# tnibler/sift-features

Hardware: AMD Instinct MI355X
Metric: keypoints+descriptors/sec on 1920×1080 batch; HBM GB/s on pyramid stage (higher is better)
Workload: dtype f32; 1 GPU; batch of 128 x 1920x1080 u8 frames per GPU (configs[3] shard), full sift(); frames_per_gpu=128, frame=1920x1080, octaves=10, parallelism=dp1 (frames sharded, no collective)

## Files before the change

### sift-features_amd/csrc/pyramid.hip

```cpp
#include "launch_ext.h"
#include "sift_common.h"
#include "sift_kernels.h"

#include <algorithm>
#include <cstdlib>
#include <cstring>

namespace siftmi {

template <int R, int TH_, int QW_ = 8>
struct BlurGeom {
    static constexpr int TW = 64;
    static constexpr int TH = TH_;
    static constexpr int QW = QW_;
    static constexpr int HWL = (R + 3) & ~3;
    static constexpr int IH = TH + 2 * R;
    static constexpr int IWV = TW + 2 * HWL;
    static constexpr int IWP = IWV + 4;
    static constexpr int OFF = HWL - R;
    static constexpr int NV = (HWL + R + QW + 3) / 4;
    static constexpr int THP = IWP;
    static constexpr int LDS_FLOATS = IH * IWP;
    static constexpr int NLOAD4 = IH * (IWV / 4);
    static constexpr int LOADS_PER_THREAD = (NLOAD4 + 255) / 256;
// ... 332 lines not shown
            const f2v kr = {taps.k[R], taps.k[R]};
            acc = v[o] * kr;
#pragma unroll
            for (int t = 1; t <= 2 * R; t++) {
                const float k = taps.k[t > R ? t - R : R - t];
                const f2v kt = {k, k};
                acc = acc + v[o + t] * kt;
            }
        }
        out[o] = acc;
    }
    const int y0 = y + WV * G::VB;
    const int nrow = min(G::VB, ye - y0);
    const int gx = x0 + 2 * lane;
    const uint32_t lane_col = (uint32_t)(gx * 4), lane_bad = gx < W ? 0u : kStoreDrop;
    const uint32_t lane_ncol = (uint32_t)((gx >> 1) * 4);
    const uint32_t lane_nbad = ((gx >> 1) < wn && (P == kProfileOpenCV || gx + 1 < W)) ? 0u : kStoreDrop;
#pragma unroll
    for (int o = 0; o < G::VB; o++) {
        const int gy = y0 + o;
        const uint32_t row_bad = o < nrow ? 0u : kStoreDrop;
        __builtin_amdgcn_raw_buffer_store_b64(__builtin_bit_cast(u32x2, out[o]), rd,
                                              ((uint32_t)(gy * pitch * 4) + lane_col) | lane_bad | row_bad, 0,
                                              SIFT_STORE_CPOL);
        if (NXT && (o & 1) == (P == kProfileOpenCV ? 0 : 1)) {
            const uint32_t nrow_bad = (gy >> 1) < hn ? row_bad : kStoreDrop;
            const uint32_t odd = __builtin_bit_cast(u32x2, out[o]).y;
            const uint32_t val = P == kProfileOpenCV
                                     ? __builtin_bit_cast(u32x2, out[o]).x
                                     : __builtin_bit_cast(uint32_t, ip_unit_clamp(__builtin_bit_cast(float, odd)));
            __builtin_amdgcn_raw_buffer_store_b32(val, rn,
                                                  ((uint32_t)((gy >> 1) * pitch_n * 4) + lane_ncol) | lane_nbad |
                                                      nrow_bad,
                                                  0, 0);
        }
    }
}

template <class G, bool NXT = false, int LOFF = 0>
__device__ __forceinline__ void strip_colpass_clamped(const float* sa, const float* sb, const BlurTaps& taps,
                                                      int lane, int wv, int y, int ye, int x0, int W, int H,
                                                      int pitch, __amdgpu_buffer_rsrc_t rd,
                                                      __amdgpu_buffer_rsrc_t rn, int pitch_n, int wn, int hn) {
    constexpr int R = G::R;
    const int y0 = y + wv * G::VB;
    const int nrow = min(G::VB, ye - y0);
    const int gx = x0 + 2 * lane;
    const uint32_t lane_col = (uint32_t)(gx * 4), lane_bad = gx < W ? 0u : kStoreDrop;
    const uint32_t lane_ncol = (uint32_t)((gx >> 1) * 4);
    const uint32_t lane_nbad = ((gx >> 1) < wn && gx + 1 < W) ? 0u : kStoreDrop;
    for (int o = 0; o < G::VB; o++) {
        const int gy = y0 + o;
        f2v acc = {0.0f, 0.0f};
#pragma unroll
        for (int t = 0; t <= 2 * R; t++) {
            const int L = min(max(gy - R + t, 0), H - 1) - (y - R - LOFF);
            const float* rp = L < G::S ? sa + L * G::IWP : sb + (L - G::S) * G::IWP;
            const f2v v = *(const lds_f2v*)(rp + 2 * lane);
            const float k = taps.k[t > R ? t - R : R - t];
            const f2v kt = {k, k};
            acc = t == 0 ? v * kt : acc + v * kt;
        }
        const uint32_t row_bad = o < nrow ? 0u : kStoreDrop;
        __builtin_amdgcn_raw_buffer_store_b64(__builtin_bit_cast(u32x2, acc), rd,
                                              ((uint32_t)(gy * pitch * 4) + lane_col) | lane_bad | row_bad, 0,
                                              SIFT_STORE_CPOL);
        if (NXT && (gy & 1) == 1) {
            const uint32_t nrow_bad = (gy >> 1) < hn ? row_bad : kStoreDrop;
            __builtin_amdgcn_raw_buffer_store_b32(__builtin_bit_cast(uint32_t, ip_unit_clamp(__builtin_bit_cast(
                                                      float, __builtin_bit_cast(u32x2, acc).y))), rn,
                                                  ((uint32_t)((gy >> 1) * pitch_n * 4) + lane_ncol) | lane_nbad |
                                                      nrow_bad,
                                                  0, 0);
        }
    }
}

#ifndef SIFT_STRIP_NXT_MINB
#define SIFT_STRIP_NXT_MINB 3
#endif
template <int R, bool NXT>
constexpr int strip_minb() {
    return (NXT && R >= 7 && StripGeom<R>::MINB > SIFT_STRIP_NXT_MINB) ? SIFT_STRIP_NXT_MINB : StripGeom<R>::MINB;
}

template <int R, int P, bool NXT>
__global__ __launch_bounds__(256, (strip_minb<R, NXT>())) void k_blur_strip(
    const float* __restrict__ src, size_t src_img_stride, float* __restrict__ dst, size_t dst_img_stride,
    float* __restrict__ nxt, size_t nxt_img_stride, int pitch_n, int wn, int hn, int W, int H, int pitch,
    const BlurTaps taps, int ya, int yb, int seg) {
    using G = StripGeom<R>;
    static_assert(G::NCW == 2, "two chunk slots");
    __shared__ __attribute__((aligned(16))) float lds[G::LDS_FLOATS];
    const int tid = threadIdx.x, lane = tid & 63;
    const int wv = __builtin_amdgcn_readfirstlane(tid >> 6);
    const TileId tile = xcd_tile();
    const int x0 = tile.x * G::TW;
    const int ys = ya + tile.y * seg, ye = min(yb, ys + seg);
    if (ys >= ye) return;
    const size_t b = tile.z;
    const uint32_t plane_bytes = (uint32_t)H * (uint32_t)pitch * 4u;
    const __amdgpu_buffer_rsrc_t rs = uniform_rsrc(src + b * src_img_stride, plane_bytes);
    const __amdgpu_buffer_rsrc_t rd = uniform_rsrc(dst + b * dst_img_stride, plane_bytes);
    __amdgpu_buffer_rsrc_t rn = rd;
    if constexpr (NXT) rn = uniform_rsrc(nxt + b * nxt_img_stride, (uint32_t)hn * (uint32_t)pitch_n * 4u);
    const bool cols_in = x0 - G::HWL >= 0 && x0 + G::TW + G::HWL <= W;
    int voff[G::LPT];
#pragma unroll
    for (int j = 0; j < G::LPT; j++) {
        const int i = min(tid + 64 * G::NW * j, G::NLOAD4 - 1);
        const int ly = i / G::C4, c4 = i - ly * G::C4;
        voff[j] = (ly * pitch + x0 - G::HWL + 4 * c4) * 4;
    }
    int prow, pq;
    strip_rowpass_map(lane, wv, prow, pq);
    const int nsteps = (ye - ys + G::S - 1) / G::S;
    float4 pre[G::LPT];
    strip_load<R, P>(pre, rs, voff, cols_in, ys - R, x0, W, H, pitch);
    strip_store<G>(pre, lds);
    strip_load<R, P>(pre, rs, voff, cols_in, ys - R + G::S, x0, W, H, pitch);
    drop_stores<G::VB * (NXT ? 2 : 1)>(rd);
    __syncthreads();
    strip_rowpass<G, P>(lds, taps, prow, pq);
    for (int k = 0; k < nsteps; k++) {
        float* sa = lds + (k & 1) * G::SLOT;
        float* sb = lds + ((k + 1) & 1) * G::SLOT;
        __syncthreads();
        strip_store<G>(pre, sb);
        if (k + 2 <= nsteps) strip_load<R, P>(pre, rs, voff, cols_in, ys - R + (k + 2) * G::S, x0, W, H, pitch);
        __syncthreads();
        strip_rowpass<G, P>(sb, taps, prow, pq);
        __syncthreads();
        const int y = ys + k * G::S;
        switch (wv) {
#define COLPASS(w)                                                                                      \
    case w:                                                                                             \
        strip_colpass<G, P, w, NXT>(sa, sb, taps, lane, y, ye, x0, W, pitch, rd, rn, pitch_n, wn, hn); \
        break;
            COLPASS(0) COLPASS(1) COLPASS(2) COLPASS(3)
            default:
                __builtin_unreachable();
#undef COLPASS
        }
    }
}

template <int Ra, int Rb, int HA = -1>
struct PairGeom {
    using GA = StripGeom<Ra, 16, HA>;
    using GB = StripGeom<Rb, 16>;
    static constexpr int HB = GB::HWL;
    static constexpr int TWO = GA::TW - 2 * HB;
    static constexpr int NBW = GB::NCW;
    static constexpr int NBR = NBW + 1;
    static constexpr int LDS_FLOATS = 2 * GA::SLOT + NBR * GB::SLOT;
    static constexpr int MINB = 163840 / (4 * LDS_FLOATS + 2048) < 4 ? 163840 / (4 * LDS_FLOATS + 2048) : 4;
    static_assert(GA::HWL <= 8 && GA::NCW == 2, "A: radius <= 8");
    static_assert(NBW == 2, "B: radius <= 8 (two-chunk column windows)");
    static_assert(GB::IWV >= GA::TW, "B's window holds A's 128 columns");
};

template <class GA, int WV, bool NXT, int P = kProfileOpenCV>
__device__ __forceinline__ void pair_colpass_a(const float* sa, const float* sb, float* bslot, int bip,
                                               const BlurTaps& taps, int lane, int y, int gys, int gye, int xa,
                                               int hb, int W, int pitch, int two, __amdgpu_buffer_rsrc_t rd,
                                               __amdgpu_buffer_rsrc_t rn, int pitch_n, int wn, int hn) {
    constexpr int R = GA::R;
    constexpr int NR = GA::VB + 2 * R;
    f2v v[NR];
#pragma unroll
    for (int j = 0; j < NR; j++) {
        const int L = WV * GA::VB + j;
        const float* rp = L < GA::S ? sa + L * GA::IWP : sb + (L - GA::S) * GA::IWP;
        v[j] = *(const lds_f2v*)(rp + 2 * lane);
    }
    const f2v k0 = {taps.k[0], taps.k[0]};
    const int y0 = y + WV * GA::VB;
    const int gx = xa + 2 * lane;
    const bool own = gx >= xa + hb && gx < xa + hb + two && gx < W;
    const uint32_t colbad = own ? 0u : kStoreDrop;

#pragma unroll
    for (int o = 0; o < GA::VB; o++) {
        f2v acc;
        if constexpr (P == kProfileOpenCV) {
            acc = v[o + R] * k0;
#pragma unroll
            for (int t = 1; t <= R; t++) {
                const f2v kt = {taps.k[t], taps.k[t]};
                acc = __builtin_elementwise_fma(v[o + R + t] + v[o + R - t], kt, acc);
            }
        } else {
            const f2v kr = {taps.k[R], taps.k[R]};
            acc = v[o] * kr;
#pragma unroll
            for (int t = 1; t <= 2 * R; t++) {
                const float k = taps.k[t > R ? t - R : R - t];
                const f2v kt = {k, k};
                acc = acc + v[o + t] * kt;
            }
        }
        *(f2v*)(bslot + (WV * GA::VB + o) * bip + 2 * lane) = acc;
        const int gy = y0 + o;
        const uint32_t rowbad = gy >= gys && gy < gye ? 0u : kStoreDrop;
        const uint32_t off = (uint32_t)((gy * pitch + gx) * 4);
        __builtin_amdgcn_raw_buffer_store_b64(__builtin_bit_cast(u32x2, acc), rd, off | colbad | rowbad, 0,
                                              SIFT_STORE_CPOL);
        if constexpr (NXT) {
            const uint32_t nbad = (gy & 1) == 0 && (gy >> 1) < hn ? rowbad : kStoreDrop;
            const uint32_t ncol = (gx >> 1) < wn ? colbad : kStoreDrop;
            __builtin_amdgcn_raw_buffer_store_b32(__builtin_bit_cast(uint32_t, acc.x), rn,
                                                  (uint32_t)(((gy >> 1) * pitch_n + (gx >> 1)) * 4) | ncol | nbad, 0,
                                                  0);
        }
    }
}

template <int Ra, int P, class GA>
struct PlaneIn {
    float4 pre[GA::LPT];
    __amdgpu_buffer_rsrc_t rs;
    int voff[GA::LPT];
    bool cols_in;
    int xa, W, H, pitch;
    __device__ __forceinline__ void init(const float* src, int xa_, int W_, int H_, int pitch_) {
        xa = xa_, W = W_, H = H_, pitch = pitch_;
        rs = uniform_rsrc(src, (uint32_t)H * (uint32_t)pitch * 4u);
        cols_in = xa - GA::HWL >= 0 && xa + GA::TW + GA::HWL <= W;
        const int tid = threadIdx.x;
#pragma unroll
        for (int j = 0; j < GA::LPT; j++) {
            const int i = min(tid + 64 * GA::NW * j, GA::NLOAD4 - 1);
            const int ly = i / GA::C4, c4 = i - ly * GA::C4;
            voff[j] = (ly * pitch + xa - GA::HWL + 4 * c4) * 4;
        }
    }
    __device__ __forceinline__ void prefetch(int r0) { strip_load<Ra, P, GA>(pre, rs, voff, cols_in, r0, xa, W, H, pitch); }
    __device__ __forceinline__ void store(float* slot, int) { strip_store<GA>(pre, slot); }
};

template <int Ra, int Rb, bool NXT, int P, bool NXTB, int LOFF, int HA, class AIn>
__device__ __forceinline__ void blur2_body(AIn& ain, float* lds, __amdgpu_buffer_rsrc_t ra, __amdgpu_buffer_rsrc_t rb,
                                           __amdgpu_buffer_rsrc_t rn, int pitch_n, int wn, int hn, int X, int ys,
                                           int ye, int W, int H, int pitch, const BlurTaps& taps_a,
                                           const BlurTaps& taps_b) {
    using Q = PairGeom<Ra, Rb, HA>;
    using GA = typename Q::GA;
    using GB = typename Q::GB;
    constexpr int S = GA::S;
    constexpr int NBW = Q::NBW, NBR = Q::NBR;
    static_assert(!(NXT && NXTB), "one next-octave output");
    float* aslot = lds;
    float* bslot = lds + 2 * GA::SLOT;
    const int tid = threadIdx.x, lane = tid & 63;
    const int wv = __builtin_amdgcn_readfirstlane(tid >> 6);
    const int xa = X - Q::HB;
    int prow, pq;
    strip_rowpass_map(lane, wv, prow, pq);
    const bool fix_l = xa < 0, fix_r = xa + GA::TW > W;
    auto fixup = [&](float* slot) {
        if (!(fix_l || fix_r)) return;
        constexpr int NE = 4 * 2 * Q::HB, NIT = (NE + 63) / 64;
        float val[NIT];
        bool act[NIT];
        int dst[NIT];
#pragma unroll
        for (int it = 0; it < NIT; it++) {
            const int e = lane + 64 * it;
            const int r = wv * 4 + e / (2 * Q::HB), j = e % (2 * Q::HB);
            const int x = j < Q::HB ? xa + j : W + (j - Q::HB);
            act[it] = e < NE && (j < Q::HB ? (fix_l && x < 0) : (fix_r && x - xa < GA::TW));
            dst[it] = r * GB::IWP + (x - xa);
            const int sx = P == kProfileOpenCV ? reflect101(x, W) : clamp_idx(x, W);
            val[it] = act[it] ? slot[r * GB::IWP + (sx - xa)] : 0.0f;
        }
        __builtin_amdgcn_fence(__ATOMIC_RELEASE, "wavefront");
        __builtin_amdgcn_wave_barrier();
#pragma unroll
        for (int it = 0; it < NIT; it++)
            if (act[it]) slot[dst[it]] = val[it];
        __builtin_amdgcn_fence(__ATOMIC_RELEASE, "wavefront");
        __builtin_amdgcn_wave_barrier();
    };
    const int nout = (ye - ys + S - 1) / S;
    const int ng = nout + NBW - 2, na = ng + 1;
    const int ga = ys - Rb - Ra - LOFF;
    ain.prefetch(ga);
    ain.store(aslot, ga);
    ain.prefetch(ga + S);
    __syncthreads();
    strip_rowpass<GA, P>(aslot, taps_a, prow, pq);
    for (int k = 0; k <= nout + NBW - 1; k++) {
        __syncthreads();
        if (k + 1 <= na) {
            ain.store(aslot + ((k + 1) & 1) * GA::SLOT, ga + (k + 1) * S);
            if (k + 2 <= na) ain.prefetch(ga + (k + 2) * S);
        }
        __syncthreads();
        if (k + 1 <= na) strip_rowpass<GA, P>(aslot + ((k + 1) & 1) * GA::SLOT, taps_a, prow, pq);
        if (k >= 1 && k - 1 <= ng) {
            float* s1 = bslot + ((k - 1) % NBR) * GB::SLOT;
            fixup(s1);
            strip_rowpass<GB, P>(s1, taps_b, prow, pq);
        }
        auto colb = [&]() {
            if (!(k >= NBW && k - NBW < nout)) return;
            const int j = k - NBW;
            const float* s0 = bslot + (j % NBR) * GB::SLOT;
            const float* s1 = bslot + ((j + 1) % NBR) * GB::SLOT;
            const int y = ys + j * S;
            if constexpr (P == kProfileImageproc) {
                const int y0 = y + wv * GB::VB;
                if (y0 - Rb < 0 || y0 + GB::VB - 1 + Rb > H - 1) {
                    if (lane < Q::TWO / 2)
                        strip_colpass_clamped<GB, NXTB, LOFF>(s0, s1, taps_b, lane, wv, y, ye, X, W, H, pitch, rb,
                                                              rn, pitch_n, wn, hn);
                    return;
                }
            }
            switch (wv) {
#define COLB(w)                                                                                                  \
    case w:                                                                                                      \
        if (lane < Q::TWO / 2)                                                                                   \
            strip_colpass<GB, P, w, NXTB, LOFF>(s0, s1, taps_b, lane, y, ye, X, W, pitch, rb, rn, pitch_n, wn, hn); \
        break;
                COLB(0) COLB(1) COLB(2) COLB(3)
                default:
                    __builtin_unreachable();
#undef COLB
            }
        };
        __syncthreads();
        if (k <= ng) {
            const float* s0 = aslot + (k & 1) * GA::SLOT;
            const float* s1 = aslot + ((k + 1) & 1) * GA::SLOT;
            float* dstb = bslot + (k % NBR) * GB::SLOT;
            const int y = ys - Rb - LOFF + k * S;
            switch (wv) {
#define COLA(w)                                                                                                       \
    case w:                                                                                                           \
        pair_colpass_a<GA, w, NXT, P>(s0, s1, dstb, GB::IWP, taps_a, lane, y, ys, ye, xa, Q::HB, W, pitch, Q::TWO, ra,\
                                   rn, pitch_n, wn, hn);                                                              \
        break;
                COLA(0) COLA(1) COLA(2) COLA(3)
                default:
                    __builtin_unreachable();
#undef COLA
            }
        }
        colb();
    }
}

template <int Ra, int Rb, bool NXT, int P = kProfileOpenCV, bool NXTB = false>
__global__ __launch_bounds__(256, (PairGeom<Ra, Rb>::MINB)) void k_blur2_strip(
    const float* __restrict__ src, size_t img_stride, float* __restrict__ dst_a, float* __restrict__ dst_b,
    float* __restrict__ nxt, size_t nxt_img_stride, int pitch_n, int wn, int hn, int W, int H, int pitch,
    const BlurTaps taps_a, const BlurTaps taps_b, int ya, int yb, int seg) {
    using Q = PairGeom<Ra, Rb>;
    static_assert(P == kProfileOpenCV || !NXT, "imageproc pairs: no next-octave output from A");
    __shared__ __attribute__((aligned(16))) float lds[Q::LDS_FLOATS];
    const TileId tile = xcd_tile();
    const int X = tile.x * Q::TWO;
    const int ys = ya + tile.y * seg, ye = min(yb, ys + seg);
    if (ys >= ye) return;
    const size_t b = tile.z;
    const uint32_t plane_bytes = (uint32_t)H * (uint32_t)pitch * 4u;
    const __amdgpu_buffer_rsrc_t ra = uniform_rsrc(dst_a + b * img_stride, plane_bytes);
    const __amdgpu_buffer_rsrc_t rb = uniform_rsrc(dst_b + b * img_stride, plane_bytes);
    __amdgpu_buffer_rsrc_t rn = ra;
    if constexpr (NXT || NXTB) rn = uniform_rsrc(nxt + b * nxt_img_stride, (uint32_t)hn * (uint32_t)pitch_n * 4u);
    PlaneIn<Ra, P, typename Q::GA> ain;
    ain.init(src + b * img_stride, X - Q::HB, W, H, pitch);
    blur2_body<Ra, Rb, NXT, P, NXTB, 0, -1>(ain, lds, ra, rb, rn, pitch_n, wn, hn, X, ys, ye, W, H, pitch, taps_a,
                                           taps_b);
}

__device__ __forceinline__ float u8_unit(uint32_t v) {
    const float fv = (float)v, c = 1.0f / 255.0f;
    const float q = fv * c;
    return __builtin_fmaf(__builtin_fmaf(-q, 255.0f, fv), c, q);
}

__device__ __forceinline__ float upsample_at(const uint8_t* __restrict__ src, size_t row_stride, int sh,
                                             const ResizeTab& tab, int dx, int dy) {
    const int sx = tab.xofs[dx];
    const bool two = dx < tab.xmax;
    const int sx1 = two ? sx + 1 : sx;
    const int sy0 = tab.yofs[dy];
    const int sy1 = sy0 + 1 < sh ? sy0 + 1 : sh - 1;
    const uint8_t* r0 = src + (size_t)sy0 * row_stride;
    const uint8_t* r1 = src + (size_t)sy1 * row_stride;
    const float p00 = u8_unit(r0[sx]), p01 = u8_unit(r0[sx1]);
    const float p10 = u8_unit(r1[sx]), p11 = u8_unit(r1[sx1]);
    const float a0 = tab.xa0[dx], a1 = tab.xa1[dx];
    const float h0 = two ? p00 * a0 + p01 * a1 : p00;
    const float h1 = two ? p10 * a0 + p11 * a1 : p10;
    return h0 * tab.ya0[dy] + h1 * tab.ya1[dy];
}

__device__ __forceinline__ void reflect_range(int p0, int n, int L, int& lo, int& hi) {
    lo = max(p0, 0);
    hi = min(p0 + n - 1, L - 1);
    if (p0 < 0) hi = max(hi, min(-p0, L - 1));
    if (p0 + n > L) lo = min(lo, max(2 * L - 1 - (p0 + n), 0));
}

template <int R, int TH>
__global__ __launch_bounds__(256) void k_seed(const uint8_t* __restrict__ frames, size_t frame_pitch,
                                              size_t row_stride, int sh, int sw, const ResizeTab tab,
                                              float* __restrict__ dst, size_t dst_img_stride, int W, int H,
                                              int pitch, const BlurTaps taps, int ty0) {
    using G = BlurGeom<R, TH>;
    constexpr int SR = G::IH / 2 + 4, SC = G::IWV / 2 + 4;
    constexpr int NW = (SC + 3) / 4 + 1;
    constexpr int NLD = (SR * NW + 255) / 256;
    __shared__ __attribute__((aligned(16))) float lds[G::LDS_FLOATS];
    __shared__ float srcf[SR * SC];
    __shared__ __attribute__((aligned(16))) float hbuf[SR * G::IWV];
    __shared__ __attribute__((aligned(16))) int txo[G::IWV];
    __shared__ __attribute__((aligned(16))) float txa0[G::IWV], txa1[G::IWV];
    __shared__ int tyo[G::IH];
    __shared__ float tya0[G::IH], tya1[G::IH];
    static_assert(G::IWV % 4 == 0 && G::IWV <= 128 && G::IH <= 128, "table threads: columns 0..127, rows 128..255");
    float* tin = lds;
    float* th = lds;
    const int tid = threadIdx.x;
    const TileId tile = xcd_tile();
    const int x0 = tile.x * G::TW, y0 = (tile.y + ty0) * G::TH;
    const size_t b = tile.z;
    const uint8_t* src = frames + b * frame_pitch;
    const bool fast = W == 2 * sw && H == 2 * sh && W >= G::IWV && H >= G::IH;
    int sxa = 0, sya = 0, sxb = -1, syb = -1;
    if (fast) {
        int glo, ghi;
        reflect_range(x0 - G::HWL, G::IWV, W, glo, ghi);
        sxa = max(glo / 2 - 1, 0);
        sxb = min(ghi / 2 + 1, sw - 1);
        reflect_range(y0 - R, G::IH, H, glo, ghi);
        sya = max(glo / 2 - 1, 0);
        syb = min(ghi / 2 + 1, sh - 1);
    }
    const int a0 = sxa & ~3;
    const int nwr = (sxb - a0) / 4 + 1, nr = syb - sya + 1;
    const bool dw_ok = (((uintptr_t)src | (uintptr_t)row_stride) & 3u) == 0;
    uint32_t wv[NLD];
#pragma unroll
    for (int j = 0; j < NLD; j++) {
        const int i = tid + 256 * j;
        const int r = i / NW, w = i - r * NW;
        wv[j] = 0;
        if (fast && r < nr && w < nwr) {
            const int c = a0 + 4 * w;
            const uint8_t* p = src + (size_t)(sya + r) * row_stride + c;
            if (c + 3 < sw && dw_ok) {
                wv[j] = *reinterpret_cast<const uint32_t*>(p);
            } else {
                for (int q = 0; q < 4 && c + q < sw; q++) wv[j] |= (uint32_t)p[q] << (8 * q);
            }
        }
    }
    {
        const int t = tid & 127;
        if (tid < 128 && t < G::IWV) {
            const int g = reflect101(x0 - G::HWL + t, W);
            const int s0 = tab.xofs[g];
            txo[t] = g < tab.xmax ? s0 : -1 - s0;
            txa0[t] = tab.xa0[g];
            txa1[t] = tab.xa1[g];
        } else if (tid >= 128 && t < G::IH) {
            const int g = reflect101(y0 - R + t, H);
            tyo[t] = tab.yofs[g];
            tya0[t] = tab.ya0[g];
            tya1[t] = tab.ya1[g];
        }
    }
    if (fast) {
#pragma unroll
        for (int j = 0; j < NLD; j++) {
            const int i = tid + 256 * j;
            const int r = i / NW, w = i - r * NW;
            if (r < nr && w < nwr) {
#pragma unroll
                for (int q = 0; q < 4; q++) {
                    const int c = a0 + 4 * w + q - sxa;
                    if (c >= 0 && c < SC) srcf[r * SC + c] = u8_unit((wv[j] >> (8 * q)) & 0xff);
                }
            }
        }
        __syncthreads();
        constexpr int Q = G::IWV / 4;
        for (int i = tid; i < nr * Q; i += 256) {
            const int r = i / Q, c = (i - r * Q) * 4;
            const int4 xo = *reinterpret_cast<const int4*>(txo + c);
            const float4 w0 = *reinterpret_cast<const float4*>(txa0 + c);
// ... 1039 lines not shown
```

### sift-features_amd/csrc/scan.hip

```cpp
#include <algorithm>
#include <type_traits>

#include "sift_common.h"
#include "sift_kernels.h"

namespace siftmi {

constexpr int DR_SH = 32;
constexpr int DR_COLS = 62;
constexpr int DR_LCAP = 256;

__device__ __forceinline__ float dpp_from_left(float v) {
    return __int_as_float(__builtin_amdgcn_mov_dpp(__float_as_int(v), 0x138, 0xf, 0xf, true));
}
__device__ __forceinline__ float dpp_from_right(float v) {
    return __int_as_float(__builtin_amdgcn_mov_dpp(__float_as_int(v), 0x130, 0xf, 0xf, true));
}

__device__ __forceinline__ uint32_t extremum3(const float (&prv)[kDogPerOctave], const float (&mid)[kDogPerOctave],
                                              const float (&cur)[kDogPerOctave], bool yin) {
    const float threshold = floorf(0.5f * kContrastThreshold / (float)kScalesPerOctave);
    float pmx[kDogPerOctave], pmn[kDogPerOctave];
#pragma unroll
    for (int p = 0; p < kDogPerOctave; p++) {
// ... 203 lines not shown
            float acc = v[0] * L.taps.k[R];
#pragma unroll
            for (int t = 1; t <= 2 * R; t++) {
                const float kt = L.taps.k[t > R ? t - R : R - t];
                acc = P == kProfileOpenCV ? __builtin_fmaf(v[t], kt, acc) : acc + v[t] * kt;
            }
            return acc;
        };
        float win[2 * R + 1];
        float prv[kDogPerOctave] = {}, mid[kDogPerOctave] = {};
        const int q0 = ya - 1 - R, q1 = yb + R;
        struct RowBuf {
            float a, c, d[4];
        };
        auto load = [&](int q, RowBuf& B, int par) {
            const int qq = min(q, q1), r = qq - R;
            ld4(qq, B.a, B.c);
            ld03(r >= ya - 1 ? min(r, yb) : ya - 1 + par, B.d);
        };
        auto shift = [&]() {
#pragma unroll
            for (int j = 0; j < 2 * R; j++) win[j] = win[j + 1];
        };
        auto step = [&](int q, const RowBuf& B, auto full_tag) {
            constexpr bool FULL = decltype(full_tag)::value;
            const bool on = FULL || q <= q1;
            const int r = q - R;
            float g5 = 0.0f;
            if (on) {
                float* wp = rg + (q & (BD_RING - 1)) * BD_RP;
                wp[lane] = B.a;
                if (lane < 2 * R) wp[64 + lane] = B.c;
                __builtin_amdgcn_fence(__ATOMIC_RELEASE, "wavefront");
                __builtin_amdgcn_wave_barrier();
                __builtin_amdgcn_fence(__ATOMIC_ACQUIRE, "wavefront");
                win[2 * R] = rowpass(q);
                if constexpr (P == kProfileOpenCV) {
                    g5 = win[R] * L.taps.k[0];
#pragma unroll
                    for (int t = 1; t <= R; t++) g5 = __builtin_fmaf(win[R + t] + win[R - t], L.taps.k[t], g5);
                } else {
                    g5 = win[0] * L.taps.k[R];
#pragma unroll
                    for (int t = 1; t <= 2 * R; t++) g5 = g5 + win[t] * L.taps.k[t > R ? t - R : R - t];
                }
            }
            const uint32_t bad = ((FULL || (on && r >= ya)) && r < yb && xst) ? 0u : 0xfffffff0u;
            __builtin_amdgcn_raw_buffer_store_b32(__builtin_bit_cast(uint32_t, g5), rg5,
                                                  ((uint32_t)(r * pitch * 4) + (uint32_t)vx) | bad, 0, 2 );
            if (!FULL && !(on && r >= ya - 1)) {
                shift();
                return;
            }
            const float g4 = rg[(r & (BD_RING - 1)) * BD_RP + lane + R];
            float cur[kDogPerOctave];
            cur[0] = B.d[1] - B.d[0];
            cur[1] = B.d[2] - B.d[1];
            cur[2] = B.d[3] - B.d[2];
            cur[3] = g4 - B.d[3];
            cur[4] = g5 - g4;
            const int y = r - 1;
            if (FULL || y >= ya) {
                const bool yin = xout && y >= kImageBorder && y < H - kImageBorder;
                uint32_t ok3 = extremum3(prv, mid, cur, yin);
                if (__ballot(ok3 != 0)) {
                    while (ok3) {
                        const int bit = __builtin_ctz(ok3);
                        ok3 &= ok3 - 1;
                        const uint64_t key = make_key((uint32_t)(L.img_base + b), (uint32_t)L.octave,
                                                      (uint32_t)(bit + 1), (uint32_t)y, (uint32_t)x);
                        const uint32_t li = atomicAdd(&lcount, 1u);
                        if (li < DR_LCAP) {
                            lcand[li] = key;
                        } else {
                            const uint32_t slot = atomicAdd(L.counter, 1u);
                            if (slot < L.cap) L.cand[slot] = key;
                        }
                    }
                }
            }
#pragma unroll
            for (int p = 0; p < kDogPerOctave; p++) {
                prv[p] = mid[p];
                mid[p] = cur[p];
            }
            shift();
        };
        RowBuf A0, A1, B0, B1;
        constexpr int GROUP = 4;
        auto group = [&](int q, auto full_tag) {
            load(q + 2, B0, 0);
            load(q + 3, B1, 1);
            __builtin_amdgcn_sched_barrier(0);
            step(q, A0, full_tag);
            step(q + 1, A1, full_tag);
            __builtin_amdgcn_sched_barrier(0);
            load(q + 4, A0, 0);
            load(q + 5, A1, 1);
            __builtin_amdgcn_sched_barrier(0);
            step(q + 2, B0, full_tag);
            step(q + 3, B1, full_tag);
            __builtin_amdgcn_sched_barrier(0);
        };
        load(q0, A0, 0);
        load(q0 + 1, A1, 1);
        int q = q0;
        for (; q < ya + R + 1; q += GROUP) group(q, std::false_type{});
        for (; q + GROUP * BD_UNROLL - 1 <= q1; q += GROUP * BD_UNROLL) {
#pragma unroll
            for (int u = 0; u < BD_UNROLL; u++) group(q + GROUP * u, std::true_type{});
        }
        for (; q <= q1; q += GROUP) group(q, std::false_type{});
    }
    __syncthreads();
    const uint32_t nl = lcount < DR_LCAP ? lcount : DR_LCAP;
    if (nl == 0) return;
    if (tid == 0) gbase = atomicAdd(L.counter, nl);
    __syncthreads();
    for (uint32_t i = tid; i < nl; i += 256)
        if (gbase + i < L.cap) L.cand[gbase + i] = lcand[i];
}

typedef float bd_f2 __attribute__((ext_vector_type(2)));
constexpr int BD2_COLS = 2 * DR_COLS;
constexpr int BD2_SLOTS = DR_COLS + 2 + 2 * 13;

struct ScanMasks {
    bool s1, s2, s3;
};
__device__ __forceinline__ ScanMasks extremum3_masks(const float (&prv)[kDogPerOctave], const float (&mid)[kDogPerOctave],
                                                     const float (&cur)[kDogPerOctave], bool yin) {
    float pmx[kDogPerOctave], pmn[kDogPerOctave];
#pragma unroll
    for (int p = 0; p < kDogPerOctave; p++) {
        const float vx = fmaxf(fmaxf(prv[p], mid[p]), cur[p]);
        const float vn = fminf(fminf(prv[p], mid[p]), cur[p]);
        const float tx = fmaxf(dpp_from_left(vx), vx), tn = fminf(dpp_from_left(vn), vn);
        pmx[p] = fmaxf(dpp_from_right(tx), tx);
        pmn[p] = fminf(dpp_from_right(tn), tn);
    }
    bool ok[kScalesPerOctave];
#pragma unroll
    for (int s_in = 1; s_in <= kScalesPerOctave; s_in++) {
        const float val = mid[s_in];
        const float mx = fmaxf(fmaxf(pmx[s_in - 1], pmx[s_in]), pmx[s_in + 1]);
        const float mn = fminf(fminf(pmn[s_in - 1], pmn[s_in]), pmn[s_in + 1]);
        const float ext = val > 0.0f ? mx : mn;
        ok[s_in - 1] = yin & (val != 0.0f) & (val == ext);
    }
    return ScanMasks{ok[0], ok[1], ok[2]};
}

#ifndef SIFT_BD2_WPE
#define SIFT_BD2_WPE 1
#endif
template <int R, int P, int NB, int U>
__global__ __launch_bounds__(256) __attribute__((amdgpu_waves_per_eu(SIFT_BD2_WPE))) void k_blur_detect_pair(
    const BlurDetectLaunch L) {
    static_assert(R <= 13 && R + 3 <= BD_RING, "ring geometry");
    __shared__ bd_f2 ring[4][BD_RING * BD2_SLOTS];
    __shared__ uint64_t lcand[DR_LCAP];
    __shared__ uint32_t lcount, gbase;
    const int tid = threadIdx.x, lane = tid & 63, wave = __builtin_amdgcn_readfirstlane(tid >> 6);
    const int W = L.W, H = L.H, pitch = L.pitch;
    const uint32_t g = xcd_block_1d() * 4 + wave;
    const uint32_t per = (uint32_t)(L.nsx * L.nsy);
    const int b = (int)(g / per);
    const uint32_t rem = g - (uint32_t)b * per;
    const int sy = (int)(rem / (uint32_t)L.nsx), sx = (int)(rem % (uint32_t)L.nsx);
    if (tid == 0) lcount = 0;
    __syncthreads();
    if (b < L.n_img) {
        const size_t P_ = (size_t)pitch * H;
        const int pb = (int)((uint32_t)P_ * 4u);
        const __amdgpu_buffer_rsrc_t rgs = uniform_rsrc(L.gauss + (size_t)b * L.img_stride, (uint32_t)(6 * pb));
        const int xb = sx * BD2_COLS;
        const int x0 = xb - 1 + lane, x1 = x0 + DR_COLS;
        const int vx0 = min(max(x0, 0), W - 1) * 4, vx1 = min(max(x1, 0), W - 1) * 4;
        const bool edge = lane >= 1 && lane <= DR_COLS;
        const bool xout0 = edge && x0 >= kImageBorder && x0 < W - kImageBorder;
        const bool xout1 = edge && x1 >= kImageBorder && x1 < W - kImageBorder;
        const uint32_t xbad0 = (edge && x0 < W) ? 0u : 0xfffffff0u, xbad1 = (edge && x1 < W) ? 0u : 0xfffffff0u;
        const int ya = sy * L.seg, yb = min(ya + L.seg, H);
        const int ca = xb - 1 - R + lane;
        const int va = bd_index<P>(ca, W) * 4, vb = bd_index<P>(ca + DR_COLS, W) * 4,
                  vc = bd_index<P>(ca + 64, W) * 4, vd = bd_index<P>(ca + 64 + DR_COLS, W) * 4;
        const bool second = lane < BD2_SLOTS - 64;
        bd_f2* rg = ring[wave];
        struct RowBuf {
            bd_f2 s0, s1;
            bd_f2 d[4];
        };
        const int q0 = ya - 1 - R, q1 = yb + R;
        auto load = [&](int q, RowBuf& B, int par) {
            const int qq = min(q, q1), r = qq - R;
            const int so = bd_index<P>(qq, H) * pitch * 4 + 4 * pb;
            B.s0 = bd_f2{buffer_load_f32(rgs, va, so), buffer_load_f32(rgs, vb, so)};
            B.s1 = bd_f2{buffer_load_f32(rgs, vc, so), buffer_load_f32(rgs, vd, so)};
            const int rr = r >= ya - 1 ? min(r, yb) : ya - 1 + par;
            const int sd = min(max(rr, 0), H - 1) * pitch * 4;
#pragma unroll
            for (int p = 0; p < 4; p++)
                B.d[p] = bd_f2{buffer_load_f32(rgs, vx0, sd + p * pb), buffer_load_f32(rgs, vx1, sd + p * pb)};
        };
        auto rowpass = [&](int q) -> bd_f2 {
            const bd_f2* p = rg + (q & (BD_RING - 1)) * BD2_SLOTS + lane;
            bd_f2 v[2 * R + 1];
#pragma unroll
            for (int t = 0; t <= 2 * R; t++) v[t] = p[t];
            bd_f2 acc = v[0] * L.taps.k[R];
#pragma unroll
            for (int t = 1; t <= 2 * R; t++) {
                const float kt = L.taps.k[t > R ? t - R : R - t];
                if constexpr (P == kProfileOpenCV)
                    acc = __builtin_elementwise_fma(v[t], (bd_f2)kt, acc);
                else
                    acc = acc + v[t] * kt;
            }
            return acc;
        };
        bd_f2 win[2 * R + 1];
        float prv0[kDogPerOctave] = {}, mid0[kDogPerOctave] = {}, prv1[kDogPerOctave] = {}, mid1[kDogPerOctave] = {};
        auto shift = [&]() {
#pragma unroll
            for (int j = 0; j < 2 * R; j++) win[j] = win[j + 1];
        };
        auto emit = [&](const ScanMasks& m, int y, int x) {
            uint32_t ok3 = (uint32_t)m.s1 | ((uint32_t)m.s2 << 1) | ((uint32_t)m.s3 << 2);
            while (ok3) {
                const int bit = __builtin_ctz(ok3);
                ok3 &= ok3 - 1;
                const uint64_t key = make_key((uint32_t)(L.img_base + b), (uint32_t)L.octave, (uint32_t)(bit + 1),
                                              (uint32_t)y, (uint32_t)x);
                const uint32_t li = atomicAdd(&lcount, 1u);
                if (li < DR_LCAP) {
                    lcand[li] = key;
                } else {
                    const uint32_t slot = atomicAdd(L.counter, 1u);
                    if (slot < L.cap) L.cand[slot] = key;
                }
            }
        };
        auto step = [&](int q, const RowBuf& B, auto full_tag) {
            constexpr bool FULL = decltype(full_tag)::value;
            const bool on = FULL || q <= q1;
            const int r = q - R;
            bd_f2 g5 = bd_f2{0.0f, 0.0f};
            if (on) {
                bd_f2* wp = rg + (q & (BD_RING - 1)) * BD2_SLOTS;
                wp[lane] = B.s0;
                if (second) wp[64 + lane] = B.s1;
                __builtin_amdgcn_fence(__ATOMIC_RELEASE, "wavefront");
                __builtin_amdgcn_wave_barrier();
                __builtin_amdgcn_fence(__ATOMIC_ACQUIRE, "wavefront");
                win[2 * R] = rowpass(q);
                if constexpr (P == kProfileOpenCV) {
                    g5 = win[R] * L.taps.k[0];
#pragma unroll
                    for (int t = 1; t <= R; t++)
                        g5 = __builtin_elementwise_fma(win[R + t] + win[R - t], (bd_f2)L.taps.k[t], g5);
                } else {
                    g5 = win[0] * L.taps.k[R];
#pragma unroll
                    for (int t = 1; t <= 2 * R; t++) g5 = g5 + win[t] * L.taps.k[t > R ? t - R : R - t];
                }
            }
            const uint32_t rbad = ((FULL || (on && r >= ya)) && r < yb) ? 0u : 0xfffffff0u;
            const int so5 = r * pitch * 4 + 5 * pb;
            const float g5x = g5.x, g5y = g5.y;
            __builtin_amdgcn_raw_buffer_store_b32(__float_as_uint(g5x), rgs, (uint32_t)vx0 | rbad | xbad0, so5,
                                                  2 );
            __builtin_amdgcn_raw_buffer_store_b32(__float_as_uint(g5y), rgs, (uint32_t)vx1 | rbad | xbad1, so5,
                                                  2 );
            if (!FULL && !(on && r >= ya - 1)) {
                shift();
                return;
            }
            const bd_f2 g4 = rg[(r & (BD_RING - 1)) * BD2_SLOTS + lane + R];
            bd_f2 cur[kDogPerOctave];
            cur[0] = B.d[1] - B.d[0];
            cur[1] = B.d[2] - B.d[1];
            cur[2] = B.d[3] - B.d[2];
            cur[3] = g4 - B.d[3];
            cur[4] = g5 - g4;
            float c0[kDogPerOctave], c1[kDogPerOctave];
#pragma unroll
            for (int p = 0; p < kDogPerOctave; p++) {
                c0[p] = cur[p].x;
                c1[p] = cur[p].y;
            }
            const int y = r - 1;
            if (FULL || y >= ya) {
                const bool yin = y >= kImageBorder && y < H - kImageBorder;
                const ScanMasks m0 = extremum3_masks(prv0, mid0, c0, yin && xout0);
                const ScanMasks m1 = extremum3_masks(prv1, mid1, c1, yin && xout1);
                if (__builtin_amdgcn_ballot_w64(m0.s1 | m0.s2 | m0.s3 | m1.s1 | m1.s2 | m1.s3)) {
                    emit(m0, y, x0);
                    emit(m1, y, x1);
                }
            }
#pragma unroll
            for (int p = 0; p < kDogPerOctave; p++) {
                prv0[p] = mid0[p];
                mid0[p] = c0[p];
                prv1[p] = mid1[p];
                mid1[p] = c1[p];
            }
            shift();
        };
        RowBuf buf[NB][2];
        constexpr int GROUP = 2 * NB;
        auto group = [&](int q, auto full_tag) {
#pragma unroll
            for (int k = 0; k < NB; k++) {
                load(q + 2 * k + 2 * (NB - 1), buf[(k + NB - 1) % NB][0], 0);
                load(q + 2 * k + 2 * (NB - 1) + 1, buf[(k + NB - 1) % NB][1], 1);
                __builtin_amdgcn_sched_barrier(0);
                step(q + 2 * k, buf[k][0], full_tag);
                step(q + 2 * k + 1, buf[k][1], full_tag);
                __builtin_amdgcn_sched_barrier(0);
            }
        };
#pragma unroll
        for (int k = 0; k < NB - 1; k++) {
            load(q0 + 2 * k, buf[k][0], 0);
            load(q0 + 2 * k + 1, buf[k][1], 1);
        }
        int q = q0;
        for (; q < ya + R + 1; q += GROUP) group(q, std::false_type{});
        if constexpr (NB == 2 && U == 3) {
            for (; q + 3 * GROUP - 1 <= q1; q += 3 * GROUP) {
                group(q, std::true_type{});
                group(q + GROUP, std::true_type{});
                group(q + 2 * GROUP, std::true_type{});
            }
        }
        for (; q + GROUP - 1 <= q1; q += GROUP) group(q, std::true_type{});
        for (; q <= q1; q += GROUP) group(q, std::false_type{});
    }
    __syncthreads();
    const uint32_t nl = lcount < DR_LCAP ? lcount : DR_LCAP;
    if (nl == 0) return;
    if (tid == 0) gbase = atomicAdd(L.counter, nl);
    __syncthreads();
    for (uint32_t i = tid; i < nl; i += 256)
        if (gbase + i < L.cap) L.cand[gbase + i] = lcand[i];
}

static bool blur_detect_pair(const BlurDetectLaunch& L, const PathOpts& o) {
    return o.bd_pair && (uint64_t)L.H * (uint64_t)L.pitch * 4 * 6 < (1ull << 31);
}

static int blur_detect_segment(int R, const BlurDetectLaunch& L, const PathOpts& o) {
    if (o.fused_detect == 0) return 0;
    const bool ok = L.W > R + 1 && L.H > R + 1 && L.W >= 2 * kImageBorder && L.H >= 2 * kImageBorder &&
                    (uint64_t)L.H * (uint64_t)L.pitch * 4 < (1ull << 31) && L.n_img > 0;
    if (!ok) return 0;
    const bool pair = blur_detect_pair(L, o);
    const bool ocv = L.profile == kProfileOpenCV;
    if (!((ocv && R == 13) || (!ocv && R == 7))) return 0;
    if (o.fused_detect == 2) return 32;
    const int cols = pair ? BD2_COLS : DR_COLS;
    const long nsx = (L.W + cols - 1) / cols;
    const long want = pair ? o.bd_waves : 16384;
    for (int s : {256, 128, 64}) {
        const int nsy = (L.H + s - 1) / s;
        if (nsx * nsy * L.n_img >= want) return (L.H + nsy - 1) / nsy;
    }
    return 0;
}

bool blur_detect_applies(int R, const BlurDetectLaunch& L, const PathOpts& o) {
    return blur_detect_segment(R, L, o) > 0;
}

int launch_blur_detect(int R, BlurDetectLaunch& L, hipStream_t st, const PathOpts& o) {
    const int seg = blur_detect_segment(R, L, o);
    if (!seg) return -1;
    const bool pair = blur_detect_pair(L, o);
    const int cols = pair ? BD2_COLS : DR_COLS;
    L.nsx = (L.W + cols - 1) / cols;
    L.seg = seg;
    L.nsy = (L.H + seg - 1) / seg;
    const long waves = (long)L.nsx * L.nsy * L.n_img;
    const dim3 grid((uint32_t)((waves + 3) / 4));
    if (pair && o.bd_pair == 2) {
        if (L.profile == kProfileOpenCV)
            hipLaunchKernelGGL((k_blur_detect_pair<13, kProfileOpenCV, 2, 1>), grid, dim3(256), 0, st, L);
        else
            hipLaunchKernelGGL((k_blur_detect_pair<7, kProfileImageproc, 2, 1>), grid, dim3(256), 0, st, L);
    } else if (pair) {
        if (L.profile == kProfileOpenCV)
            hipLaunchKernelGGL((k_blur_detect_pair<13, kProfileOpenCV, 2, 3>), grid, dim3(256), 0, st, L);
        else
            hipLaunchKernelGGL((k_blur_detect_pair<7, kProfileImageproc, 2, 3>), grid, dim3(256), 0, st, L);
    } else if (L.profile == kProfileOpenCV)
        hipLaunchKernelGGL((k_blur_detect<13, kProfileOpenCV>), grid, dim3(256), 0, st, L);
    else
        hipLaunchKernelGGL((k_blur_detect<7, kProfileImageproc>), grid, dim3(256), 0, st, L);
    return 0;
}

}
```

Before: 37.90 million keypoints/s.

## Hold pair A-pass results in registers and restructure blur-detect pipeline

The pair blur kernel now keeps the A column-pass outputs in registers and writes them into the B slot at the start of the next iteration. This lets the B ring shrink by one LDS slot, lowering LDS use per block to raise occupancy. In blur_detect_pair the row pass loads taps in chunks behind a compiler barrier, the row buffering becomes a 3-deep single-row ring with step-then-load order and 4x unrolling, and waves-per-EU moves from 1 to 3. The launch variants for the bd_pair modes collapse into one. This risks more register pressure and hazards from reusing the slot with fewer buffers.

```diff
diff --git a/sift-features_amd/csrc/pyramid.hip b/sift-features_amd/csrc/pyramid.hip
--- a/sift-features_amd/csrc/pyramid.hip
+++ b/sift-features_amd/csrc/pyramid.hip
@@ -508,7 +508,7 @@
     static constexpr int HB = GB::HWL;
     static constexpr int TWO = GA::TW - 2 * HB;
     static constexpr int NBW = GB::NCW;
-    static constexpr int NBR = NBW + 1;
+    static constexpr int NBR = NBW;
     static constexpr int LDS_FLOATS = 2 * GA::SLOT + NBR * GB::SLOT;
     static constexpr int MINB = 163840 / (4 * LDS_FLOATS + 2048) < 4 ? 163840 / (4 * LDS_FLOATS + 2048) : 4;
     static_assert(GA::HWL <= 8 && GA::NCW == 2, "A: radius <= 8");
@@ -517,7 +517,7 @@
 };
 
 template <class GA, int WV, bool NXT, int P = kProfileOpenCV>
-__device__ __forceinline__ void pair_colpass_a(const float* sa, const float* sb, float* bslot, int bip,
+__device__ __forceinline__ void pair_colpass_a(const float* sa, const float* sb, f2v (&keep)[GA::VB],
                                                const BlurTaps& taps, int lane, int y, int gys, int gye, int xa,
                                                int hb, int W, int pitch, int two, __amdgpu_buffer_rsrc_t rd,
                                                __amdgpu_buffer_rsrc_t rn, int pitch_n, int wn, int hn) {
@@ -556,7 +556,7 @@
                 acc = acc + v[o + t] * kt;
             }
         }
-        *(f2v*)(bslot + (WV * GA::VB + o) * bip + 2 * lane) = acc;
+        keep[o] = acc;
         const int gy = y0 + o;
         const uint32_t rowbad = gy >= gys && gy < gye ? 0u : kStoreDrop;
         const uint32_t off = (uint32_t)((gy * pitch + gx) * 4);
@@ -641,6 +641,8 @@
     const int nout = (ye - ys + S - 1) / S;
     const int ng = nout + NBW - 2, na = ng + 1;
     const int ga = ys - Rb - Ra - LOFF;
+    f2v keep[GA::VB] = {};
+    float* const kdst = bslot + (wv * GA::VB) * GB::IWP + 2 * lane;
     ain.prefetch(ga);
     ain.store(aslot, ga);
     ain.prefetch(ga + S);
@@ -648,6 +650,11 @@
     strip_rowpass<GA, P>(aslot, taps_a, prow, pq);
     for (int k = 0; k <= nout + NBW - 1; k++) {
         __syncthreads();
+        if (k >= 1) {
+#pragma unroll
+            for (int o = 0; o < GA::VB; o++)
+                *(f2v*)(kdst + ((k - 1) % NBR) * GB::SLOT + o * GB::IWP) = keep[o];
+        }
         if (k + 1 <= na) {
             ain.store(aslot + ((k + 1) & 1) * GA::SLOT, ga + (k + 1) * S);
             if (k + 2 <= na) ain.prefetch(ga + (k + 2) * S);
@@ -690,13 +697,12 @@
         if (k <= ng) {
             const float* s0 = aslot + (k & 1) * GA::SLOT;
             const float* s1 = aslot + ((k + 1) & 1) * GA::SLOT;
-            float* dstb = bslot + (k % NBR) * GB::SLOT;
             const int y = ys - Rb - LOFF + k * S;
             switch (wv) {
 #define COLA(w)                                                                                                       \
     case w:                                                                                                           \
-        pair_colpass_a<GA, w, NXT, P>(s0, s1, dstb, GB::IWP, taps_a, lane, y, ys, ye, xa, Q::HB, W, pitch, Q::TWO, ra,\
-                                   rn, pitch_n, wn, hn);                                                              \
+        pair_colpass_a<GA, w, NXT, P>(s0, s1, keep, taps_a, lane, y, ys, ye, xa, Q::HB, W, pitch, Q::TWO, ra, rn,    \
+                                      pitch_n, wn, hn);                                                               \
         break;
                 COLA(0) COLA(1) COLA(2) COLA(3)
                 default:
diff --git a/sift-features_amd/csrc/scan.hip b/sift-features_amd/csrc/scan.hip
--- a/sift-features_amd/csrc/scan.hip
+++ b/sift-features_amd/csrc/scan.hip
@@ -379,9 +379,12 @@
 }
 
 #ifndef SIFT_BD2_WPE
-#define SIFT_BD2_WPE 1
+#define SIFT_BD2_WPE 3
 #endif
-template <int R, int P, int NB, int U>
+#ifndef BD2_TAPS
+#define BD2_TAPS 4
+#endif
+template <int R, int P>
 __global__ __launch_bounds__(256) __attribute__((amdgpu_waves_per_eu(SIFT_BD2_WPE))) void k_blur_detect_pair(
     const BlurDetectLaunch L) {
     static_assert(R <= 13 && R + 3 <= BD_RING, "ring geometry");
@@ -432,17 +435,26 @@
         };
         auto rowpass = [&](int q) -> bd_f2 {
             const bd_f2* p = rg + (q & (BD_RING - 1)) * BD2_SLOTS + lane;
-            bd_f2 v[2 * R + 1];
-#pragma unroll
-            for (int t = 0; t <= 2 * R; t++) v[t] = p[t];
-            bd_f2 acc = v[0] * L.taps.k[R];
-#pragma unroll
-            for (int t = 1; t <= 2 * R; t++) {
-                const float kt = L.taps.k[t > R ? t - R : R - t];
-                if constexpr (P == kProfileOpenCV)
-                    acc = __builtin_elementwise_fma(v[t], (bd_f2)kt, acc);
-                else
-                    acc = acc + v[t] * kt;
+            constexpr int NT = 2 * R + 1;
+            bd_f2 v[NT];
+#pragma unroll
+            for (int t = 0; t < BD2_TAPS && t < NT; t++) v[t] = p[t];
+            bd_f2 acc = bd_f2{0.0f, 0.0f};
+#pragma unroll
+            for (int t0 = 0; t0 < NT; t0 += BD2_TAPS) {
+#pragma unroll
+                for (int t = t0 + BD2_TAPS; t < t0 + 2 * BD2_TAPS && t < NT; t++) v[t] = p[t];
+#pragma unroll
+                for (int t = t0; t < t0 + BD2_TAPS && t < NT; t++) {
+                    const float kt = L.taps.k[t > R ? t - R : R - t];
+                    if (t == 0)
+                        acc = v[0] * kt;
+                    else if constexpr (P == kProfileOpenCV)
+                        acc = __builtin_elementwise_fma(v[t], (bd_f2)kt, acc);
+                    else
+                        acc = acc + v[t] * kt;
+                }
+                if (t0 + 2 * BD2_TAPS < NT) asm volatile("" : "+v"(acc)::"memory");
             }
             return acc;
         };
@@ -454,6 +466,7 @@
         };
         auto emit = [&](const ScanMasks& m, int y, int x) {
             uint32_t ok3 = (uint32_t)m.s1 | ((uint32_t)m.s2 << 1) | ((uint32_t)m.s3 << 2);
+            asm volatile("" : "+v"(x));
             while (ok3) {
                 const int bit = __builtin_ctz(ok3);
                 ok3 &= ok3 - 1;
@@ -535,32 +548,24 @@
             }
             shift();
         };
-        RowBuf buf[NB][2];
-        constexpr int GROUP = 2 * NB;
+        RowBuf buf[3];
+        constexpr int GROUP = 3;
         auto group = [&](int q, auto full_tag) {
 #pragma unroll
-            for (int k = 0; k < NB; k++) {
-                load(q + 2 * k + 2 * (NB - 1), buf[(k + NB - 1) % NB][0], 0);
-                load(q + 2 * k + 2 * (NB - 1) + 1, buf[(k + NB - 1) % NB][1], 1);
+            for (int k = 0; k < GROUP; k++) {
+                step(q + k, buf[k], full_tag);
                 __builtin_amdgcn_sched_barrier(0);
-                step(q + 2 * k, buf[k][0], full_tag);
-                step(q + 2 * k + 1, buf[k][1], full_tag);
+                load(q + k + GROUP, buf[k], k & 1);
                 __builtin_amdgcn_sched_barrier(0);
             }
         };
 #pragma unroll
-        for (int k = 0; k < NB - 1; k++) {
-            load(q0 + 2 * k, buf[k][0], 0);
-            load(q0 + 2 * k + 1, buf[k][1], 1);
-        }
+        for (int k = 0; k < GROUP; k++) load(q0 + k, buf[k], k & 1);
         int q = q0;
         for (; q < ya + R + 1; q += GROUP) group(q, std::false_type{});
-        if constexpr (NB == 2 && U == 3) {
-            for (; q + 3 * GROUP - 1 <= q1; q += 3 * GROUP) {
-                group(q, std::true_type{});
-                group(q + GROUP, std::true_type{});
-                group(q + 2 * GROUP, std::true_type{});
-            }
+        for (; q + 4 * GROUP - 1 <= q1; q += 4 * GROUP) {
+#pragma unroll
+            for (int u = 0; u < 4; u++) group(q + u * GROUP, std::true_type{});
         }
         for (; q + GROUP - 1 <= q1; q += GROUP) group(q, std::true_type{});
         for (; q <= q1; q += GROUP) group(q, std::false_type{});
@@ -611,16 +616,11 @@
     L.nsy = (L.H + seg - 1) / seg;
     const long waves = (long)L.nsx * L.nsy * L.n_img;
     const dim3 grid((uint32_t)((waves + 3) / 4));
-    if (pair && o.bd_pair == 2) {
+    if (pair) {
         if (L.profile == kProfileOpenCV)
-            hipLaunchKernelGGL((k_blur_detect_pair<13, kProfileOpenCV, 2, 1>), grid, dim3(256), 0, st, L);
+            hipLaunchKernelGGL((k_blur_detect_pair<13, kProfileOpenCV>), grid, dim3(256), 0, st, L);
         else
-            hipLaunchKernelGGL((k_blur_detect_pair<7, kProfileImageproc, 2, 1>), grid, dim3(256), 0, st, L);
-    } else if (pair) {
-        if (L.profile == kProfileOpenCV)
-            hipLaunchKernelGGL((k_blur_detect_pair<13, kProfileOpenCV, 2, 3>), grid, dim3(256), 0, st, L);
-        else
-            hipLaunchKernelGGL((k_blur_detect_pair<7, kProfileImageproc, 2, 3>), grid, dim3(256), 0, st, L);
+            hipLaunchKernelGGL((k_blur_detect_pair<7, kProfileImageproc>), grid, dim3(256), 0, st, L);
     } else if (L.profile == kProfileOpenCV)
         hipLaunchKernelGGL((k_blur_detect<13, kProfileOpenCV>), grid, dim3(256), 0, st, L);
     else
```

Result: faster. 39.18 million keypoints/s, median of 6 (+3.4%).
